# GPUs/goVideoCompressor

Measured on AMD Instinct MI355X. Metric: encoded frames/sec (whole node), 1080p30->H.264 CRF23, higher is better.
Workload: dtype uint8 (8-bit 4:2:0 samples, int32 transforms)

## Files before the change

### csrc/common/h264_cabac.h

```cpp
#pragma once
#include <cstddef>
#include <cstdint>

#include "h264_cabac_tables.h"
#include "h264_mb.h"
#include "h264_tables.h"

namespace mivc {
namespace h264 {

#if defined(__HIPCC__) && defined(__HIP_DEVICE_COMPILE__)
MIVC_HD int cabac_clz32(uint32_t v) { return __clz(static_cast<int>(v)); }
#else
MIVC_HD int cabac_clz32(uint32_t v) { return v ? __builtin_clz(v) : 32; }
#endif

struct CabacBuf {
  uint8_t* p;
  size_t cap;
  size_t n;
  int overflow;
  MIVC_HD void put(int b) {
    if (n < cap) p[n] = static_cast<uint8_t>(b);
    else overflow = 1;
// ... 453 lines not shown
    if (!((cbp >> b8) & 1)) continue;
    const int x4 = (b8 & 1) * 2, y4 = (b8 >> 1) * 2;
    if (n.t8x8) {
      n.cbf_luma |= static_cast<uint16_t>(0x33u << (x4 + 4 * y4));
      continue;
    }
    for (int b4 = 0; b4 < 4; ++b4) {
      const int blk = b8 * 4 + b4;
      if ((mask >> blk) & 1u) n.cbf_luma |= static_cast<uint16_t>(1u << (kBlkX[blk] + 4 * kBlkY[blk]));
    }
  }
}

MIVC_HD void cabac_qp_chain(const CabacSliceInfo& si, CabacNb* nb, int n) {
  int last_qp = si.slice_qp, last_nz = 0;
  for (int a = si.first_mb; a < si.first_mb + n; ++a) {
    CabacNb& m = nb[a];
    const bool has = !m.skip && (m.cbp != 0 || m.kind == MBK_I16x16);
    m.prev_dqp_nz = static_cast<uint8_t>(last_nz);
    if (has) {
      int d = m.qp - last_qp;
      if (d < -26) d += 52;
      if (d > 25) d -= 52;
      m.dqp = static_cast<int8_t>(d);
      last_qp = m.qp;
      last_nz = d != 0;
    } else {
      m.dqp = 0;
      last_nz = 0;
    }
  }
}

template <class E>
struct CabacMbCoder {
  E& e;
  const CabacSliceInfo& si;
  const CabacNb* nb;
  CabacView v;
  const CabacNb* cur;

  MIVC_HD CabacMbCoder(E& e_, const CabacSliceInfo& s, const CabacNb* table) : e(e_), si(s), nb(table), cur(nullptr) {}

  MIVC_HD const CabacNb* nb_mb(int x4, int y4) const {
    const int a = v.mb_of(x4, y4);
    return a < 0 ? nullptr : &nb[a];
  }
  MIVC_HD const CabacNb* A() const { return nb_mb(-1, 0); }
  MIVC_HD const CabacNb* B() const { return nb_mb(0, -1); }

  MIVC_HD void put_mb_skip(int skip) {
    const CabacNb* a = A();
    const CabacNb* b = B();
    const int inc = (a && !a->skip) + (b && !b->skip);
    e.decision((si.slice_type == SLICE_B ? CTX_MB_SKIP_B : CTX_MB_SKIP_P) + inc, skip);
  }

  MIVC_HD void put_mb_type_i(int kind, int i16_mode, int cbp, bool islice) {
    if (islice) {
      const CabacNb* a = A();
      const CabacNb* b = B();
      const int inc = (a && a->kind != MBK_I4x4 && a->kind != MBK_I8x8) + (b && b->kind != MBK_I4x4 && b->kind != MBK_I8x8);
      e.decision(CTX_MB_TYPE_I + inc, kind == MBK_I4x4 || kind == MBK_I8x8 ? 0 : 1);
    } else {
      const int off = si.slice_type == SLICE_B ? CTX_MB_TYPE_B_INTRA : CTX_MB_TYPE_P_INTRA;
      e.decision(off, kind == MBK_I4x4 || kind == MBK_I8x8 ? 0 : 1);
    }
    if (kind == MBK_I4x4 || kind == MBK_I8x8) return;
    e.terminate(kind == MBK_IPCM ? 1 : 0);
    if (kind == MBK_IPCM) return;
    const int cl = (cbp & 15) ? 1 : 0, cc = cbp >> 4;
    if (islice) {
      e.decision(CTX_MB_TYPE_I + 3, cl);
      e.decision(CTX_MB_TYPE_I + 4, cc != 0);
      if (cc) e.decision(CTX_MB_TYPE_I + 5, cc == 2);
      e.decision(CTX_MB_TYPE_I + 6, (i16_mode >> 1) & 1);
      e.decision(CTX_MB_TYPE_I + 7, i16_mode & 1);
    } else {
      const int off = si.slice_type == SLICE_B ? CTX_MB_TYPE_B_INTRA : CTX_MB_TYPE_P_INTRA;
      e.decision(off + 1, cl);
      e.decision(off + 2, cc != 0);
      if (cc) e.decision(off + 2, cc == 2);
      e.decision(off + 3, (i16_mode >> 1) & 1);
      e.decision(off + 3, i16_mode & 1);
    }
  }

  MIVC_HD void put_mb_type_p(int kind, int i16_mode, int cbp) {
    switch (kind) {
      case MBK_P16x16: e.decision(14, 0); e.decision(15, 0); e.decision(16, 0); return;
      case MBK_P16x8:  e.decision(14, 0); e.decision(15, 1); e.decision(17, 1); return;
      case MBK_P8x16:  e.decision(14, 0); e.decision(15, 1); e.decision(17, 0); return;
      case MBK_P8x8:   e.decision(14, 0); e.decision(15, 0); e.decision(16, 1); return;
      default:
        e.decision(14, 1);
        put_mb_type_i(kind, i16_mode, cbp, false);
    }
  }

  MIVC_HD void put_mb_type_b(int kind, int i16_mode, int cbp, int code) {
    const CabacNb* a = A();
    const CabacNb* b = B();
    const int inc = (a && !a->skip && a->kind != MBK_BDIRECT) + (b && !b->skip && b->kind != MBK_BDIRECT);
    if (code == 0) {
      e.decision(CTX_MB_TYPE_B + inc, 0);
      return;
    }
    e.decision(CTX_MB_TYPE_B + inc, 1);
    if (code <= 2) {
      e.decision(CTX_MB_TYPE_B + 3, 0);
      e.decision(CTX_MB_TYPE_B + 5, code - 1);
      return;
    }
    e.decision(CTX_MB_TYPE_B + 3, 1);
    if (code <= 10) {
      const int v3 = code - 3;
      e.decision(CTX_MB_TYPE_B + 4, 0);
      e.decision(CTX_MB_TYPE_B + 5, (v3 >> 2) & 1);
      e.decision(CTX_MB_TYPE_B + 5, (v3 >> 1) & 1);
      e.decision(CTX_MB_TYPE_B + 5, v3 & 1);
      return;
    }
    e.decision(CTX_MB_TYPE_B + 4, 1);
    if (code == 11 || code == 22 || code == 23) {
      e.decision(CTX_MB_TYPE_B + 5, 1);
      e.decision(CTX_MB_TYPE_B + 5, code == 23 ? 0 : 1);
      e.decision(CTX_MB_TYPE_B + 5, code == 11 ? 0 : 1);
      if (code == 23) put_mb_type_i(kind, i16_mode, cbp, false);
      return;
    }
    const int v4 = code - 12;
    e.decision(CTX_MB_TYPE_B + 5, (v4 >> 3) & 1);
    e.decision(CTX_MB_TYPE_B + 5, (v4 >> 2) & 1);
    e.decision(CTX_MB_TYPE_B + 5, (v4 >> 1) & 1);
    e.decision(CTX_MB_TYPE_B + 5, v4 & 1);
  }

  MIVC_HD void put_sub_mb_type_b(int code) {
    if (code == 0) { e.decision(CTX_SUB_MB_B, 0); return; }
    e.decision(CTX_SUB_MB_B, 1);
    if (code <= 2) {
      e.decision(CTX_SUB_MB_B + 1, 0);
      e.decision(CTX_SUB_MB_B + 3, code - 1);
      return;
    }
    e.decision(CTX_SUB_MB_B + 1, 1);
    if (code <= 6) {
      e.decision(CTX_SUB_MB_B + 2, 0);
      e.decision(CTX_SUB_MB_B + 3, ((code - 3) >> 1) & 1);
      e.decision(CTX_SUB_MB_B + 3, (code - 3) & 1);
      return;
    }
    e.decision(CTX_SUB_MB_B + 2, 1);
    if (code >= 11) {
      e.decision(CTX_SUB_MB_B + 3, 1);
      e.decision(CTX_SUB_MB_B + 3, code - 11);
      return;
    }
    e.decision(CTX_SUB_MB_B + 3, 0);
    e.decision(CTX_SUB_MB_B + 3, ((code - 7) >> 1) & 1);
    e.decision(CTX_SUB_MB_B + 3, (code - 7) & 1);
  }

  MIVC_HD void put_ref_idx(int list, int q, int ref) {
    const int x4 = (q & 1) * 2, y4 = (q >> 1) * 2;
    auto cond = [&](int xn, int yn) -> int {
      const CabacNb* m = nb_mb(xn, yn);
      if (!m || m->skip || mbk_is_intra(m->kind)) return 0;
      const int qn = CabacView::quad_of(xn, yn);
      if ((m->direct >> qn) & 1) return 0;
      return m->ref[list][qn] > 0;
    };
    const int inc = cond(x4 - 1, y4) + 2 * cond(x4, y4 - 1);
    e.decision(CTX_REF_IDX + inc, ref > 0);
    if (ref == 0) return;
    for (int k = 1; k < ref; ++k) e.decision(CTX_REF_IDX + (k == 1 ? 4 : 5), 1);
    e.decision(CTX_REF_IDX + (ref == 1 ? 4 : 5), 0);
  }

  MIVC_HD void put_mvd(int list, int q, int comp, int val) {
    const int x4 = (q & 1) * 2, y4 = (q >> 1) * 2;
    auto absn = [&](int xn, int yn) -> int {
      const CabacNb* m = nb_mb(xn, yn);
      if (!m) return 0;
      const int d = m->mvd[list][CabacView::quad_of(xn, yn)][comp];
      return d < 0 ? -d : d;
    };
    const int sum = absn(x4 - 1, y4) + absn(x4, y4 - 1);
    const int base = comp ? CTX_MVD_Y : CTX_MVD_X;
    const int inc0 = sum < 3 ? 0 : (sum > 32 ? 2 : 1);
    const int av = val < 0 ? -val : val;
    const int pre = av < 9 ? av : 9;
    e.decision(base + inc0, pre > 0);
    if (pre > 0) {
      for (int k = 1; k < pre; ++k) e.decision(base + (k < 4 ? k + 2 : 6), 1);
      if (pre < 9) e.decision(base + (pre < 4 ? pre + 2 : 6), 0);
      if (av >= 9) e.bypass_eg(static_cast<uint32_t>(av - 9), 3);
      e.bypass(val < 0);
    }
  }

  MIVC_HD void put_cbp(int cbp) {
    const CabacNb* a = A();
    const CabacNb* b = B();
    const int la = a ? (a->kind == MBK_IPCM ? 0x2F : a->cbp) : 0x0F;
    const int lb = b ? (b->kind == MBK_IPCM ? 0x2F : b->cbp) : 0x0F;
    for (int b8 = 0; b8 < 4; ++b8) {
      const int ca = (b8 & 1) ? ((cbp >> (b8 - 1)) & 1) : ((la >> (b8 + 1)) & 1);
      const int cb = (b8 & 2) ? ((cbp >> (b8 - 2)) & 1) : ((lb >> (b8 + 2)) & 1);
      e.decision(CTX_CBP_LUMA + (ca ? 0 : 1) + 2 * (cb ? 0 : 1), (cbp >> b8) & 1);
    }
    const int ca = a ? (a->kind == MBK_IPCM ? 2 : (a->cbp >> 4)) : 0;
    const int cb = b ? (b->kind == MBK_IPCM ? 2 : (b->cbp >> 4)) : 0;
    const int cc = cbp >> 4;
    e.decision(CTX_CBP_CHROMA + (ca > 0) + 2 * (cb > 0), cc > 0);
    if (cc) e.decision(CTX_CBP_CHROMA + 4 + (ca == 2) + 2 * (cb == 2), cc == 2);
  }

  MIVC_HD void put_qp_delta(int d, int prev_nz) {
    const int m = d > 0 ? 2 * d - 1 : -2 * d;
    e.decision(CTX_QP_DELTA + (prev_nz ? 1 : 0), m > 0);
    if (m > 0) {
      for (int k = 1; k < m; ++k) e.decision(CTX_QP_DELTA + (k == 1 ? 2 : 3), 1);
      e.decision(CTX_QP_DELTA + (m == 1 ? 2 : 3), 0);
    }
  }

  MIVC_HD void put_chroma_mode(int mode) {
    const CabacNb* a = A();
    const CabacNb* b = B();
    const int inc = (a && mbk_is_intra(a->kind) && a->kind != MBK_IPCM && a->chroma_mode != 0) +
                    (b && mbk_is_intra(b->kind) && b->kind != MBK_IPCM && b->chroma_mode != 0);
    e.decision(CTX_CHROMA_PRED + inc, mode > 0);
    if (mode > 0) {
      e.decision(CTX_CHROMA_PRED + 3, mode > 1);
      if (mode > 1) e.decision(CTX_CHROMA_PRED + 3, mode > 2);
    }
  }

  MIVC_HD int pred_intra_mode(int x4, int y4) const {
    const CabacNb* a = nb_mb(x4 - 1, y4);
    const CabacNb* b = nb_mb(x4, y4 - 1);
    if (!a || !b) return 2;
    const int ma = (a->kind == MBK_I4x4 || a->kind == MBK_I8x8) ? a->i4[CabacView::rast_of(x4 - 1, y4)] : 2;
    const int mb = (b->kind == MBK_I4x4 || b->kind == MBK_I8x8) ? b->i4[CabacView::rast_of(x4, y4 - 1)] : 2;
    return ma < mb ? ma : mb;
  }
  MIVC_HD void put_intra_mode(int mode, int pred) {
    if (mode == pred) {
      e.decision(CTX_PREV_INTRA, 1);
      return;
    }
    e.decision(CTX_PREV_INTRA, 0);
    const int rem = mode < pred ? mode : mode - 1;
    e.decision(CTX_REM_INTRA, rem & 1);
    e.decision(CTX_REM_INTRA, (rem >> 1) & 1);
    e.decision(CTX_REM_INTRA, (rem >> 2) & 1);
  }

  MIVC_HD void put_t8x8(int flag) {
    const CabacNb* a = A();
    const CabacNb* b = B();
    e.decision(CTX_T8x8 + (a && a->t8x8) + (b && b->t8x8), flag);
  }

  MIVC_HD void put_block(const int16_t* c, int n, int cat, int cbf_inc, bool nonzero) {
    if (!nonzero) {
      if (cbf_inc >= 0) e.decision(CTX_CBF + kCbfCatOffset[cat] + cbf_inc, 0);
      return;
    }
    int last = -1;
    for (int i = 0; i < n; ++i)
      if (c[i]) last = i;
    if (cbf_inc >= 0) {
      e.decision(CTX_CBF + kCbfCatOffset[cat] + cbf_inc, last >= 0);
      if (last < 0) return;
    }
    for (int i = 0; i < n - 1; ++i) {
      const int sig = c[i] != 0;
      int sctx, lctx;
      if (cat == 5) {
        sctx = CTX_SIG8x8 + kSig8x8Frame[i];
        lctx = CTX_LAST8x8 + kLast8x8Frame[i];
      } else {
        const int inc = cat == 3 ? (i < 2 ? i : 2) : i;
        sctx = CTX_SIG + kSigCatOffset[cat] + inc;
        lctx = CTX_LAST + kSigCatOffset[cat] + inc;
      }
      e.decision(sctx, sig);
      if (sig) {
        e.decision(lctx, i == last);
        if (i == last) break;
      }
    }
    const int abase = cat == 5 ? CTX_ABS8x8 : CTX_ABS + kAbsCatOffset[cat];
    const int gmax = cat == 3 ? 3 : 4;
    int ngt1 = 0, neq1 = 0;
    for (int i = last; i >= 0; --i) {
      const int val = c[i];
      if (!val) continue;
      const int a1 = (val < 0 ? -val : val) - 1;
      e.decision(abase + (ngt1 ? 0 : (neq1 + 1 < 4 ? neq1 + 1 : 4)), a1 > 0);
      if (a1 > 0) {
        const int ctx1 = abase + 5 + (ngt1 < gmax ? ngt1 : gmax);
        const int pre = a1 < 14 ? a1 : 14;
        for (int k = 1; k < pre; ++k) e.decision(ctx1, 1);
        if (pre < 14) e.decision(ctx1, 0);
        else e.bypass_eg(static_cast<uint32_t>(a1 - 14), 0);
        ++ngt1;
      } else {
        ++neq1;
      }
      e.bypass(val < 0);
    }
  }

  MIVC_HD int cbf_luma_inc(int x4, int y4, bool intra) const {
    auto cond = [&](int xn, int yn) -> int {
      const CabacNb* m = nb_mb(xn, yn);
      if (!m) return intra ? 1 : 0;
      if (m->kind == MBK_IPCM) return 1;
      return (m->cbf_luma >> CabacView::rast_of(xn, yn)) & 1;
    };
    return cond(x4 - 1, y4) + 2 * cond(x4, y4 - 1);
  }
  MIVC_HD int cbf_dc_inc(int bit, bool intra) const {
    auto cond = [&](const CabacNb* m) -> int {
      if (!m) return intra ? 1 : 0;
      if (m->kind == MBK_IPCM) return 1;
      return (m->cbf_dc >> bit) & 1;
    };
    return cond(A()) + 2 * cond(B());
  }
  MIVC_HD int cbf_cac_inc(int comp, int cx, int cy, bool intra) const {
    auto cond = [&](const CabacNb* m, int blk) -> int {
      if (!m) return intra ? 1 : 0;
      if (m->kind == MBK_IPCM) return 1;
      return (m->cbf_cac[comp] >> blk) & 1;
    };
    const int a = cx > 0 ? cond(cur, cy * 2) : cond(A(), cy * 2 + 1);
    const int b = cy > 0 ? cond(cur, cx) : cond(B(), 2 + cx);
    return a + 2 * b;
  }

  MIVC_HD void put_inter_pred(const MbHeader& h, int kind) {
    if (kind == MBK_BDIRECT) return;
    const bool bslice = si.slice_type == SLICE_B;
    const CabacParts P = cabac_parts(kind);
    const bool sub8 = P.np == 4;
    const int dir_mask = cur->direct;
    if (sub8) {
      if (bslice) {
        for (int s = 0; s < 4; ++s) {
          int code = 0;
          if (!((dir_mask >> s) & 1)) {
            const bool l0 = h.ref[0][s] >= 0, l1 = h.ref[1][s] >= 0;
            code = (l0 && l1) ? 3 : (l1 ? 2 : 1);
          }
          put_sub_mb_type_b(code);
        }
      } else {
        for (int s = 0; s < 4; ++s) e.decision(CTX_SUB_MB_P, 1);
      }
    }
    for (int l = 0; l < 2; ++l) {
      if (si.num_ref[l] <= 1) continue;
      for (int p = 0; p < P.np; ++p) {
        const int q = P.qfirst(p);
        if (((dir_mask >> q) & 1) || h.ref[l][q] < 0) continue;
        put_ref_idx(l, q, h.ref[l][q]);
      }
    }
    for (int l = 0; l < 2; ++l)
      for (int p = 0; p < P.np; ++p) {
        const int q = P.qfirst(p);
        if (((dir_mask >> q) & 1) || h.ref[l][q] < 0) continue;
        put_mvd(l, q, 0, cur->mvd[l][q][0]);
        put_mvd(l, q, 1, cur->mvd[l][q][1]);
      }
  }

  MIVC_HD void code_mb(int addr, const MbHeader& h, const int16_t* c, bool last_in_slice) {
    v.at(addr, si.wmb, si.first_mb);
    cur = &nb[addr];
    const bool pslice = si.slice_type == SLICE_P, bslice = si.slice_type == SLICE_B;
    if (pslice || bslice) put_mb_skip(cur->skip);
    if (!cur->skip) code_mb_layer(h, c);
    e.terminate(last_in_slice ? 1 : 0);
  }

  MIVC_HD void code_mb_layer(const MbHeader& h, const int16_t* c) {
    const bool pslice = si.slice_type == SLICE_P, bslice = si.slice_type == SLICE_B;
    const int kind = cur->kind;
    const int cbp = cur->cbp;
    const uint32_t mask = cur->mask;
    const bool intra = mbk_is_intra(kind);
    if (pslice) put_mb_type_p(kind, h.i16_mode, cbp);
    else if (bslice) put_mb_type_b(kind, h.i16_mode, cbp, intra ? 23 : cur->b_code);
    else put_mb_type_i(kind, h.i16_mode, cbp, true);
    if (kind == MBK_I4x4 || kind == MBK_I8x8) {
      if (si.t8x8_mode) put_t8x8(kind == MBK_I8x8);
      if (kind == MBK_I4x4) {
        for (int blk = 0; blk < 16; ++blk) {
          const int x4 = kBlkX[blk], y4 = kBlkY[blk];
          put_intra_mode(h.i4_modes[blk], pred_intra_mode(x4, y4));
        }
      } else {
        for (int b8 = 0; b8 < 4; ++b8) put_intra_mode(h.i4_modes[b8 * 4], pred_intra_mode((b8 & 1) * 2, (b8 >> 1) * 2));
      }
    }
    if (intra) put_chroma_mode(h.chroma_mode);
    else put_inter_pred(h, kind);
    if (kind != MBK_I16x16) {
      put_cbp(cbp);
      if ((cbp & 15) && si.t8x8_mode && !intra) put_t8x8(cur->t8x8);
    }
    if (cbp == 0 && kind != MBK_I16x16) return;
    put_qp_delta(cur->dqp, cur->prev_dqp_nz);
    if (kind == MBK_I16x16) put_block(c + COEF_LUMA_DC, 16, 0, cbf_dc_inc(0, true), (mask & NZ_LUMA_DC) != 0);
    for (int b8 = 0; b8 < 4; ++b8) {
      if (!((cbp >> b8) & 1)) continue;
      if (cur->t8x8) {
        put_block(c + COEF_LUMA + b8 * 64, 64, 5, -1, true);
        continue;
      }
      for (int b4 = 0; b4 < 4; ++b4) {
        const int blk = b8 * 4 + b4;
        const int inc = cbf_luma_inc(kBlkX[blk], kBlkY[blk], intra);
        const bool nzb = (mask >> blk) & 1u;
        if (kind == MBK_I16x16) put_block(c + COEF_LUMA + blk * 16 + 1, 15, 1, inc, nzb);
        else put_block(c + COEF_LUMA + blk * 16, 16, 2, inc, nzb);
      }
    }
    const int cc = cbp >> 4;
    if (cc)
      for (int comp = 0; comp < 2; ++comp)
        put_block(c + COEF_CHROMA_DC + comp * 4, 4, 3, cbf_dc_inc(1 + comp, intra), ((mask >> (17 + comp)) & 1u) != 0);
    if (cc == 2)
      for (int comp = 0; comp < 2; ++comp)
        for (int b = 0; b < 4; ++b)
          put_block(c + COEF_CHROMA_AC + (comp * 4 + b) * 16 + 1, 15, 4, cbf_cac_inc(comp, b & 1, b >> 1, intra),
                    ((mask >> (19 + comp * 4 + b)) & 1u) != 0);
  }
};

MIVC_HD void cabac_code_symbol(CabacEncoder& e, uint16_t s) {
  if (!(s & 0x8000u)) e.decision(s & 0x1FF, (s >> 9) & 1);
  else if (!(s & 0x4000u)) e.bypass_bits(s & 0x3FFu, (s >> 10) & 15);
  else e.terminate(s & 1);
}

template <class Out>
struct CabacSymbolCoder {
  uint64_t low;
  uint32_t range;
  int nbits, bad;
  Out out;

  MIVC_HD void init() {
    low = 0;
    range = 510;
    nbits = -1;
    bad = 0;
  }
  MIVC_HD void drain() {
    while (nbits >= 8) {
      const int sh = nbits + 2;
      const uint32_t v = static_cast<uint32_t>(low >> sh);
      low &= (1ull << sh) - 1ull;
      nbits -= 8;
      if (!out.byte9(v)) bad = 1;
    }
  }
  MIVC_HD void step_nodrain(uint32_t sym, uint8_t* st, int stride, const uint8_t* lps, const uint8_t* trans) {
// ... 156 lines not shown
```

### csrc/kernels/bindings_hip.cc

```cpp
#include <pybind11/pybind11.h>
#include <pybind11/stl.h>

#include <cstdint>
#include <stdexcept>
#include <string>
#include <vector>

#include "../common/hevc_ctu_coder.h"
#include "launch.h"
#include "route.h"

namespace py = pybind11;
using mivc::gpu::kExactMaxRows;
using mivc::gpu::kMaxCols;
using mivc::gpu::kMaxRows;

namespace {
template <class T>
T* P(uintptr_t p) {
  return reinterpret_cast<T*>(p);
}
void* S(uintptr_t s) { return reinterpret_cast<void*>(s); }

void limit(const char* entry, const char* what, int n, int most) {
// ... 673 lines not shown
    a.ctb_ops = P<uint32_t>(Q("ctb_ops"));
    a.refs = P<uint8_t>(Q("refs"));
    a.ref_base = P<int32_t>(Q("ref_base"));
    a.slices = P<uint8_t>(Q("slices"));
    a.slice_base = P<int32_t>(Q("slice_base"));
    a.scaling = P<uint8_t>(Q("scaling"));
    a.max_tus = static_cast<int>(I("max_tus"));
    a.err = P<int>(Q("err"));
    if (p.contains("out")) {
      const std::vector<uintptr_t> out = p["out"].cast<std::vector<uintptr_t>>();
      for (int c = 0; c < 3; ++c) a.out[c] = reinterpret_cast<void*>(out.at(c));
      a.out_u8 = static_cast<int>(I("out_u8"));
      a.Fo = static_cast<int>(I("Fo"));
      a.out_w = static_cast<int>(I("out_w"));
      a.out_h = static_cast<int>(I("out_h"));
      a.crop_x = static_cast<int>(I("crop_x"));
      a.crop_y = static_cast<int>(I("crop_y"));
      a.disp = P<int16_t>(Q("disp"));
    }
    if (!a.cur || !a.run || !a.meta || !a.mvf || !a.err) throw std::runtime_error("hevc_decode_stage: null pointer");
    const int r = mivc_launch_hevc_decode(&a, stage, S(stream));
    if (r != 0) throw std::runtime_error("hevc_decode_stage: launch failed (" + std::to_string(r) + ")");
  });
  m.def("cavlc_mb_bytes", []() { return mivc_cavlc_mb_bytes(); });
  m.def("cabac_nb_bytes", []() { return mivc_cabac_nb_bytes(); });
  m.def("cabac_gap", []() { return mivc_cabac_gap(); });
  m.def("cabac_bin", [](int B, int wmb, int hmb, uintptr_t hdr, uintptr_t coef, uintptr_t mask, uintptr_t nb,
                        uintptr_t cnt, uintptr_t off, uintptr_t tot, uintptr_t pool, long long pool_cap,
                        uintptr_t pool_used, uintptr_t base, uintptr_t total, uintptr_t slot_qp, int slice_type,
                        int num_ref_l0, int num_ref_l1, int t8x8_mode, uintptr_t err, uintptr_t stream, uintptr_t route,
                        int slice_rows, uintptr_t pre) {
    if (pre && !route) throw std::invalid_argument("cabac_bin: pre needs the step's route");
    if ((pool & 15) != 0) throw std::invalid_argument("cabac_bin: symbol pool must be 16-byte aligned");
    if (B < 1 || wmb < 1 || hmb < 1) throw std::invalid_argument("cabac_bin: bad geometry");
    mivc_launch_cabac_bin(B, wmb, hmb, P<void>(hdr), P<int16_t>(coef), P<uint32_t>(mask), P<void>(nb), P<int>(cnt),
                          P<long long>(off), P<int>(tot), P<uint16_t>(pool), pool_cap, P<long long>(pool_used),
                          P<long long>(base), P<int>(total), P<int>(slot_qp), slice_type, num_ref_l0, num_ref_l1,
                          t8x8_mode, P<int>(err), S(stream), P<void>(route), slice_rows, P<uint32_t>(pre));
  }, py::arg("B"), py::arg("wmb"), py::arg("hmb"), py::arg("hdr"), py::arg("coef"), py::arg("mask"), py::arg("nb"),
     py::arg("cnt"), py::arg("off"), py::arg("tot"), py::arg("pool"), py::arg("pool_cap"), py::arg("pool_used"),
     py::arg("base"), py::arg("total"), py::arg("slot_qp"), py::arg("slice_type"), py::arg("num_ref_l0"),
     py::arg("num_ref_l1"), py::arg("t8x8_mode"), py::arg("err"), py::arg("stream"), py::arg("route") = 0,
     py::arg("slice_rows") = 0, py::arg("pre") = 0);
  m.def("cabac_code", [](int L, int B, uintptr_t pool, uintptr_t base, uintptr_t total, uintptr_t hdr_bits,
                         uintptr_t hdr_nbits, uintptr_t slot_qp, unsigned long long itypes, uintptr_t bytes,
                         uintptr_t out, uintptr_t out_off, uintptr_t err, uintptr_t stream, uintptr_t host_out,
                         long long host_cap) {
    if (B < 1 || L < 1 || L % B != 0 || L / B > 64) throw std::invalid_argument("cabac_code: L must be G * B, G <= 64");
    if ((out & 15) || (host_out & 15)) throw std::invalid_argument("cabac_code: output buffers must be 16-byte aligned");
    mivc_launch_cabac_code(L, B, P<uint16_t>(pool), P<long long>(base), P<int>(total), P<uint32_t>(hdr_bits),
                           P<int>(hdr_nbits), P<int>(slot_qp), itypes, P<int>(bytes), P<uint8_t>(out),
                           P<long long>(out_off), P<int>(err), P<uint8_t>(host_out), host_cap, S(stream));
  });
  m.def("cavlc", [](int B, int wmb, int hmb, uintptr_t hdr, uintptr_t coef, uintptr_t mbs, uintptr_t len, uintptr_t off,
                    uintptr_t trail, uintptr_t total_bits, uintptr_t slot_bytes, uintptr_t words, long long cap_words,
                    uintptr_t hdr_bits, uintptr_t hdr_nbits, int pslice, int slice_qp, uintptr_t slot_qp,
                    uintptr_t out, uintptr_t out_off, uintptr_t stream, uintptr_t nz) {
    mivc_launch_cavlc(B, wmb, hmb, P<void>(hdr), P<int16_t>(coef), P<void>(mbs), P<int>(len), P<long long>(off),
                      P<int>(trail), P<long long>(total_bits), P<int>(slot_bytes), P<uint32_t>(words), cap_words,
                      P<uint32_t>(hdr_bits), P<int>(hdr_nbits), pslice, slice_qp, P<int>(slot_qp), P<uint8_t>(out),
                      P<long long>(out_off), P<uint8_t>(nz), S(stream));
  }, py::arg("B"), py::arg("wmb"), py::arg("hmb"), py::arg("hdr"), py::arg("coef"), py::arg("mbs"), py::arg("len"),
     py::arg("off"), py::arg("trail"), py::arg("total_bits"), py::arg("slot_bytes"), py::arg("words"),
     py::arg("cap_words"), py::arg("hdr_bits"), py::arg("hdr_nbits"), py::arg("pslice"), py::arg("slice_qp"),
     py::arg("slot_qp"), py::arg("out"), py::arg("out_off"), py::arg("stream"), py::arg("nz") = 0);
  m.def("sse", [](int B, int W, int H, int w, int h, uintptr_t sy, uintptr_t su, uintptr_t sv, uintptr_t ry,
// ... 41 lines not shown
```

### csrc/kernels/cabac.hip

```cpp
#include "kcommon.h"
#include "launch.h"
#include "../common/h264_cabac.h"

namespace mivc {
namespace gpu {

using h264::CabacNb;
using h264::CabacSliceInfo;
using h264::MbHeader;

constexpr int kCabacGap = 64;
constexpr int kArithReadAhead = 160;

struct CabacBinArgs {
  Geom g;
  const MbHeader* hdr;
  const int16_t* coef;
  uint32_t* mask;
  CabacNb* nb;
  int* cnt;
  long long* off;
  int* tot;
  uint16_t* pool;
  long long pool_cap;
// ... 163 lines not shown
  for (int i = i0; i < i1; ++i) loc += a.cnt[base + i];
  const long long incl = wave_scan_add(loc);
  long long p = incl - loc;
  for (int i = i0; i < i1; ++i) {
    a.off[base + i] = p;
    p += a.cnt[base + i];
  }
  if (lane == 63) a.tot[blockIdx.x] = static_cast<int>(incl);
}

__global__ __launch_bounds__(64) void cabac_alloc(CabacBinArgs a) {
  const int B = a.g.B * a.per_slot, lane = threadIdx.x;
  const int per = (B + 63) / 64;
  const int i0 = lane * per, i1 = min(B, i0 + per);
  auto region = [&](int s) { return (static_cast<long long>(a.tot[s]) + kCabacGap + 7) & ~7ll; };
  long long loc = 0;
  for (int i = i0; i < i1; ++i) loc += region(i);
  const long long incl = wave_scan_add(loc);
  const long long sum = __shfl(incl, 63, 64);
  long long p = incl - loc;
  const long long start = *a.pool_used;
  const bool fits = start + sum + kArithReadAhead <= a.pool_cap;
  for (int i = i0; i < i1; ++i) {
    a.base[i] = start + p;
    a.total[i] = fits ? a.tot[i] : -1;
    p += region(i);
  }
  if (lane == 0) {
    if (fits) *a.pool_used = start + sum;
    else atomicOr(a.err, 4);
  }
}

struct StagedEmit {
  uint16_t* g;
  uint16_t* lds;
  long long start;
  long long pos;
  int n;
  __device__ __forceinline__ void emit(uint16_t s) {
    lds[pos & 7] = s;
    ++pos;
    ++n;
    if ((pos & 7) == 0) {
      const long long c0 = pos - 8;
      if (c0 >= start) {
        const uint32_t* w = reinterpret_cast<const uint32_t*>(lds);
        *reinterpret_cast<uint4*>(g + c0) = make_uint4(w[0], w[1], w[2], w[3]);
      } else {
        for (long long i = start; i < pos; ++i) g[i] = lds[i & 7];
      }
    }
  }
  __device__ __forceinline__ void finish() {
    const long long c0 = pos & ~7ll;
    for (long long i = c0 > start ? c0 : start; i < pos; ++i) g[i] = lds[i & 7];
  }
};

__global__ __launch_bounds__(64) __attribute__((amdgpu_waves_per_eu(6, 8))) void cabac_bins(CabacBinArgs a) {
  __shared__ __attribute__((aligned(16))) uint16_t stage[64 * 8];
  const int mb = blockIdx.x * 64 + threadIdx.x, slot = blockIdx.y, n = a.g.nmb();
  if (mb >= n) return;
  const int ls = slice_index(a, slot, mb);
  if (a.total[ls] < 0) return;
  const CabacSliceInfo si = slice_info(a, slot, mb);
  const size_t base = static_cast<size_t>(slot) * n;
  h264::CabacSymbolPacker<StagedEmit> s;
  s.out.g = a.pool + a.base[ls] + kCabacGap;
  s.out.lds = stage + threadIdx.x * 8;
  s.out.start = s.out.pos = a.off[base + mb];
  s.out.n = 0;
  h264::CabacMbCoder<h264::CabacSymbolPacker<StagedEmit>> coder(s, si, a.nb + base);
  coder.code_mb(mb, a.hdr[base + mb], a.coef + (base + mb) * h264::kCoefPerMb, mb == slice_end(a, mb) - 1);
  s.flush_bypass();
  s.out.finish();
}

struct CabacCodeArgs {
  int L;
  int B;
  int lpw;
  uint16_t* pool;
  const long long* base;
  const int* total;
  const uint32_t* hdr_bits;
  const int* hdr_nbits;
  const int* slot_qp;
  unsigned long long itypes;
  int* bytes;
  uint8_t* out;
  long long* out_off;
  int* err;
  uint8_t* host_out;
  long long host_cap;
};

struct RingOut {
  uint8_t* p;
  uint8_t* ring;
  long long n, flushed, cap;
  long long arith0;
  long long hold;
  int ovf;
  __device__ void start(long long header_bytes) {
    arith0 = header_bytes;
    hold = -1;
  }
  __device__ void flush_words() {
// ... 271 lines not shown
```

Before: 17690.

## Vectorize CABAC neighbor and coefficient loads, drop LDS staging for symbol emits

Neighbor macroblock context is loaded once per MB as 16-byte heads into registers instead of repeated byte loads through pointers. Coefficient blocks are loaded as wide vectors and turned into a nonzero bitmap that drives the significance and level loops, with packed nibble tables for 8x8 contexts. The LDS-staged 16-byte symbol writer is replaced by plain per-symbol global stores. This trades scattered scalar loads and LDS traffic for more registers and uncoalesced 2-byte stores, and adds alignment requirements on coef and nb.

Result: no change. 17830 (median of 2 runs) (+0.8%).

```diff
diff --git a/csrc/common/h264_cabac.h b/csrc/common/h264_cabac.h
--- a/csrc/common/h264_cabac.h
+++ b/csrc/common/h264_cabac.h
@@ -509,6 +509,109 @@
   }
 }
 
+MIVC_HD uint32_t cabac_load32(const void* p) {
+#if defined(__HIPCC__) && defined(__HIP_DEVICE_COMPILE__)
+  return *static_cast<const uint32_t*>(p);
+#else
+  uint32_t v;
+  __builtin_memcpy(&v, p, 4);
+  return v;
+#endif
+}
+
+struct CabacLevelWindow {
+  uint32_t w0, w1, w2, w3, w4, w5, w6, w7;
+  MIVC_HD void load16(const int16_t* row) {
+#if defined(__HIPCC__) && defined(__HIP_DEVICE_COMPILE__)
+    const uint4 a = reinterpret_cast<const uint4*>(row)[0];
+    const uint4 b = reinterpret_cast<const uint4*>(row)[1];
+    w0 = a.x; w1 = a.y; w2 = a.z; w3 = a.w;
+    w4 = b.x; w5 = b.y; w6 = b.z; w7 = b.w;
+#else
+    uint32_t t[8];
+    __builtin_memcpy(t, row, 32);
+    w0 = t[0]; w1 = t[1]; w2 = t[2]; w3 = t[3];
+    w4 = t[4]; w5 = t[5]; w6 = t[6]; w7 = t[7];
+#endif
+  }
+  MIVC_HD void load4(const int16_t* quad) {
+#if defined(__HIPCC__) && defined(__HIP_DEVICE_COMPILE__)
+    const uint2 a = *reinterpret_cast<const uint2*>(quad);
+    w0 = a.x; w1 = a.y;
+#else
+    uint32_t t[2];
+    __builtin_memcpy(t, quad, 8);
+    w0 = t[0]; w1 = t[1];
+#endif
+    w2 = w3 = w4 = w5 = w6 = w7 = 0;
+  }
+  static MIVC_HD uint32_t nz2(uint32_t w) { return ((w & 0xFFFFu) ? 1u : 0u) | ((w >> 16) ? 2u : 0u); }
+  MIVC_HD uint32_t nzmap() const {
+    return nz2(w0) | (nz2(w1) << 2) | (nz2(w2) << 4) | (nz2(w3) << 6) | (nz2(w4) << 8) | (nz2(w5) << 10) |
+           (nz2(w6) << 12) | (nz2(w7) << 14);
+  }
+  MIVC_HD int level(int i) const {
+    const uint32_t a0 = (i & 2) ? w1 : w0, a1 = (i & 2) ? w3 : w2, a2 = (i & 2) ? w5 : w4, a3 = (i & 2) ? w7 : w6;
+    const uint32_t b0 = (i & 4) ? a1 : a0, b1 = (i & 4) ? a3 : a2;
+    const uint32_t c = (i & 8) ? b1 : b0;
+    return static_cast<int16_t>((i & 1) ? (c >> 16) : (c & 0xFFFFu));
+  }
+};
+
+constexpr uint64_t cabac_pack_nibbles(const uint8_t* t, int first, int n) {
+  uint64_t v = 0;
+  for (int i = 0; i < 16 && first + i < n; ++i) v |= static_cast<uint64_t>(t[first + i] & 15u) << (4 * i);
+  return v;
+}
+MIVC_HD int cabac_nibble_row(int i, uint64_t r0, uint64_t r1, uint64_t r2, uint64_t r3) {
+  const uint64_t a = (i & 16) ? r1 : r0, b = (i & 16) ? r3 : r2;
+  return static_cast<int>((((i & 32) ? b : a) >> (4 * (i & 15))) & 15u);
+}
+MIVC_HD int cabac_sig8x8_inc(int i) {
+  constexpr uint64_t r0 = cabac_pack_nibbles(kSig8x8Frame, 0, 63), r1 = cabac_pack_nibbles(kSig8x8Frame, 16, 63),
+                     r2 = cabac_pack_nibbles(kSig8x8Frame, 32, 63), r3 = cabac_pack_nibbles(kSig8x8Frame, 48, 63);
+  return cabac_nibble_row(i, r0, r1, r2, r3);
+}
+MIVC_HD int cabac_last8x8_inc(int i) {
+  constexpr uint64_t r0 = cabac_pack_nibbles(kLast8x8Frame, 0, 63), r1 = cabac_pack_nibbles(kLast8x8Frame, 16, 63),
+                     r2 = cabac_pack_nibbles(kLast8x8Frame, 32, 63), r3 = cabac_pack_nibbles(kLast8x8Frame, 48, 63);
+  return cabac_nibble_row(i, r0, r1, r2, r3);
+}
+
+struct CabacNbHead {
+  uint32_t w0, w1, w2, w3;
+  bool ok;
+  MIVC_HD void load(const CabacNb* m, bool present) {
+#if defined(__HIPCC__) && defined(__HIP_DEVICE_COMPILE__)
+    const uint4 a = *reinterpret_cast<const uint4*>(m);
+    w0 = a.x; w1 = a.y; w2 = a.z; w3 = a.w;
+#else
+    uint32_t t[4];
+    __builtin_memcpy(t, m, 16);
+    w0 = t[0]; w1 = t[1]; w2 = t[2]; w3 = t[3];
+#endif
+    ok = present;
+  }
+  MIVC_HD int kind() const { return (w0 >> 8) & 0xFF; }
+  MIVC_HD int skip() const { return (w0 >> 16) & 0xFF; }
+  MIVC_HD int cbp() const { return w0 >> 24; }
+  MIVC_HD int t8x8() const { return w1 & 0xFF; }
+  MIVC_HD int chroma_mode() const { return (w1 >> 8) & 0xFF; }
+  MIVC_HD int direct() const { return (w1 >> 16) & 0xFF; }
+  MIVC_HD int cbf_dc() const { return w1 >> 24; }
+  MIVC_HD int cbf_luma() const { return w2 & 0xFFFF; }
+  MIVC_HD int cbf_cac(int comp) const { return (w2 >> (16 + 8 * comp)) & 0xFF; }
+};
+static_assert(offsetof(CabacNb, kind) == 1 && offsetof(CabacNb, skip) == 2 && offsetof(CabacNb, cbp) == 3 &&
+                  offsetof(CabacNb, t8x8) == 4 && offsetof(CabacNb, chroma_mode) == 5 &&
+                  offsetof(CabacNb, direct) == 6 && offsetof(CabacNb, cbf_dc) == 7 &&
+                  offsetof(CabacNb, cbf_luma) == 8 && offsetof(CabacNb, cbf_cac) == 10 &&
+                  offsetof(CabacNb, ref) == 12 && offsetof(CabacNb, mvd) % 4 == 0 && offsetof(CabacNb, i16_mode) % 4 == 0 &&
+                  offsetof(CabacNb, b_code) == offsetof(CabacNb, i16_mode) + 1 &&
+                  offsetof(CabacNb, dqp) == offsetof(CabacNb, i16_mode) + 2 &&
+                  offsetof(CabacNb, prev_dqp_nz) == offsetof(CabacNb, i16_mode) + 3 && sizeof(CabacNb) % 16 == 0,
+              "CabacNbHead decodes the leading 16 bytes of CabacNb (little-endian)");
+
 template <class E>
 struct CabacMbCoder {
   E& e;
@@ -516,6 +619,7 @@
   const CabacNb* nb;
   CabacView v;
   const CabacNb* cur;
+  CabacNbHead hc, ha, hb;
 
   MIVC_HD CabacMbCoder(E& e_, const CabacSliceInfo& s, const CabacNb* table) : e(e_), si(s), nb(table), cur(nullptr) {}
 
@@ -523,21 +627,17 @@
     const int a = v.mb_of(x4, y4);
     return a < 0 ? nullptr : &nb[a];
   }
-  MIVC_HD const CabacNb* A() const { return nb_mb(-1, 0); }
-  MIVC_HD const CabacNb* B() const { return nb_mb(0, -1); }
+  MIVC_HD CabacNbHead head_of(int x4, int y4) const { return x4 < 0 ? ha : (y4 < 0 ? hb : hc); }
 
   MIVC_HD void put_mb_skip(int skip) {
-    const CabacNb* a = A();
-    const CabacNb* b = B();
-    const int inc = (a && !a->skip) + (b && !b->skip);
+    const int inc = (ha.ok && !ha.skip()) + (hb.ok && !hb.skip());
     e.decision((si.slice_type == SLICE_B ? CTX_MB_SKIP_B : CTX_MB_SKIP_P) + inc, skip);
   }
 
   MIVC_HD void put_mb_type_i(int kind, int i16_mode, int cbp, bool islice) {
     if (islice) {
-      const CabacNb* a = A();
-      const CabacNb* b = B();
-      const int inc = (a && a->kind != MBK_I4x4 && a->kind != MBK_I8x8) + (b && b->kind != MBK_I4x4 && b->kind != MBK_I8x8);
+      const int inc = (ha.ok && ha.kind() != MBK_I4x4 && ha.kind() != MBK_I8x8) +
+                      (hb.ok && hb.kind() != MBK_I4x4 && hb.kind() != MBK_I8x8);
       e.decision(CTX_MB_TYPE_I + inc, kind == MBK_I4x4 || kind == MBK_I8x8 ? 0 : 1);
     } else {
       const int off = si.slice_type == SLICE_B ? CTX_MB_TYPE_B_INTRA : CTX_MB_TYPE_P_INTRA;
@@ -576,9 +676,7 @@
   }
 
   MIVC_HD void put_mb_type_b(int kind, int i16_mode, int cbp, int code) {
-    const CabacNb* a = A();
-    const CabacNb* b = B();
-    const int inc = (a && !a->skip && a->kind != MBK_BDIRECT) + (b && !b->skip && b->kind != MBK_BDIRECT);
+    const int inc = (ha.ok && !ha.skip() && ha.kind() != MBK_BDIRECT) + (hb.ok && !hb.skip() && hb.kind() != MBK_BDIRECT);
     if (code == 0) {
       e.decision(CTX_MB_TYPE_B + inc, 0);
       return;
@@ -642,11 +740,13 @@
   MIVC_HD void put_ref_idx(int list, int q, int ref) {
     const int x4 = (q & 1) * 2, y4 = (q >> 1) * 2;
     auto cond = [&](int xn, int yn) -> int {
-      const CabacNb* m = nb_mb(xn, yn);
-      if (!m || m->skip || mbk_is_intra(m->kind)) return 0;
+      const CabacNbHead m = head_of(xn, yn);
+      const int a = v.mb_of(xn, yn);
+      const uint32_t row = list == 0 ? m.w3 : cabac_load32(&nb[a < 0 ? v.addr : a].ref[1][0]);
+      if (!m.ok || m.skip() || mbk_is_intra(m.kind())) return 0;
       const int qn = CabacView::quad_of(xn, yn);
-      if ((m->direct >> qn) & 1) return 0;
-      return m->ref[list][qn] > 0;
+      if ((m.direct() >> qn) & 1) return 0;
+      return static_cast<int8_t>((row >> (8 * qn)) & 0xFFu) > 0;
     };
     const int inc = cond(x4 - 1, y4) + 2 * cond(x4, y4 - 1);
     e.decision(CTX_REF_IDX + inc, ref > 0);
@@ -655,15 +755,22 @@
     e.decision(CTX_REF_IDX + (ref == 1 ? 4 : 5), 0);
   }
 
-  MIVC_HD void put_mvd(int list, int q, int comp, int val) {
+  MIVC_HD void put_mvd_pair(int list, int q) {
     const int x4 = (q & 1) * 2, y4 = (q >> 1) * 2;
-    auto absn = [&](int xn, int yn) -> int {
-      const CabacNb* m = nb_mb(xn, yn);
-      if (!m) return 0;
-      const int d = m->mvd[list][CabacView::quad_of(xn, yn)][comp];
-      return d < 0 ? -d : d;
+    auto pair = [&](int xn, int yn) -> uint32_t {
+      const int a = v.mb_of(xn, yn);
+      const uint32_t d = cabac_load32(&nb[a < 0 ? v.addr : a].mvd[list][CabacView::quad_of(xn, yn)][0]);
+      return a < 0 ? 0u : d;
     };
-    const int sum = absn(x4 - 1, y4) + absn(x4, y4 - 1);
+    const uint32_t own = cabac_load32(&cur->mvd[list][q][0]);
+    const uint32_t l = pair(x4 - 1, y4), t = pair(x4, y4 - 1);
+    auto comp_of = [](uint32_t d, int comp) -> int { return static_cast<int16_t>(comp ? (d >> 16) : (d & 0xFFFFu)); };
+    auto mag = [](int d) -> int { return d < 0 ? -d : d; };
+    for (int comp = 0; comp < 2; ++comp)
+      put_mvd(comp, comp_of(own, comp), mag(comp_of(l, comp)) + mag(comp_of(t, comp)));
+  }
+
+  MIVC_HD void put_mvd(int comp, int val, int sum) {
     const int base = comp ? CTX_MVD_Y : CTX_MVD_X;
     const int inc0 = sum < 3 ? 0 : (sum > 32 ? 2 : 1);
     const int av = val < 0 ? -val : val;
@@ -678,17 +785,15 @@
   }
 
   MIVC_HD void put_cbp(int cbp) {
-    const CabacNb* a = A();
-    const CabacNb* b = B();
-    const int la = a ? (a->kind == MBK_IPCM ? 0x2F : a->cbp) : 0x0F;
-    const int lb = b ? (b->kind == MBK_IPCM ? 0x2F : b->cbp) : 0x0F;
+    const int la = ha.ok ? (ha.kind() == MBK_IPCM ? 0x2F : ha.cbp()) : 0x0F;
+    const int lb = hb.ok ? (hb.kind() == MBK_IPCM ? 0x2F : hb.cbp()) : 0x0F;
     for (int b8 = 0; b8 < 4; ++b8) {
       const int ca = (b8 & 1) ? ((cbp >> (b8 - 1)) & 1) : ((la >> (b8 + 1)) & 1);
       const int cb = (b8 & 2) ? ((cbp >> (b8 - 2)) & 1) : ((lb >> (b8 + 2)) & 1);
       e.decision(CTX_CBP_LUMA + (ca ? 0 : 1) + 2 * (cb ? 0 : 1), (cbp >> b8) & 1);
     }
-    const int ca = a ? (a->kind == MBK_IPCM ? 2 : (a->cbp >> 4)) : 0;
-    const int cb = b ? (b->kind == MBK_IPCM ? 2 : (b->cbp >> 4)) : 0;
+    const int ca = ha.ok ? (ha.kind() == MBK_IPCM ? 2 : (ha.cbp() >> 4)) : 0;
+    const int cb = hb.ok ? (hb.kind() == MBK_IPCM ? 2 : (hb.cbp() >> 4)) : 0;
     const int cc = cbp >> 4;
     e.decision(CTX_CBP_CHROMA + (ca > 0) + 2 * (cb > 0), cc > 0);
     if (cc) e.decision(CTX_CBP_CHROMA + 4 + (ca == 2) + 2 * (cb == 2), cc == 2);
@@ -704,10 +809,8 @@
   }
 
   MIVC_HD void put_chroma_mode(int mode) {
-    const CabacNb* a = A();
-    const CabacNb* b = B();
-    const int inc = (a && mbk_is_intra(a->kind) && a->kind != MBK_IPCM && a->chroma_mode != 0) +
-                    (b && mbk_is_intra(b->kind) && b->kind != MBK_IPCM && b->chroma_mode != 0);
+    const int inc = (ha.ok && mbk_is_intra(ha.kind()) && ha.kind() != MBK_IPCM && ha.chroma_mode() != 0) +
+                    (hb.ok && mbk_is_intra(hb.kind()) && hb.kind() != MBK_IPCM && hb.chroma_mode() != 0);
     e.decision(CTX_CHROMA_PRED + inc, mode > 0);
     if (mode > 0) {
       e.decision(CTX_CHROMA_PRED + 3, mode > 1);
@@ -736,46 +839,15 @@
   }
 
   MIVC_HD void put_t8x8(int flag) {
-    const CabacNb* a = A();
-    const CabacNb* b = B();
-    e.decision(CTX_T8x8 + (a && a->t8x8) + (b && b->t8x8), flag);
-  }
-
-  MIVC_HD void put_block(const int16_t* c, int n, int cat, int cbf_inc, bool nonzero) {
-    if (!nonzero) {
-      if (cbf_inc >= 0) e.decision(CTX_CBF + kCbfCatOffset[cat] + cbf_inc, 0);
-      return;
-    }
-    int last = -1;
-    for (int i = 0; i < n; ++i)
-      if (c[i]) last = i;
-    if (cbf_inc >= 0) {
-      e.decision(CTX_CBF + kCbfCatOffset[cat] + cbf_inc, last >= 0);
-      if (last < 0) return;
-    }
-    for (int i = 0; i < n - 1; ++i) {
-      const int sig = c[i] != 0;
-      int sctx, lctx;
-      if (cat == 5) {
-        sctx = CTX_SIG8x8 + kSig8x8Frame[i];
-        lctx = CTX_LAST8x8 + kLast8x8Frame[i];
-      } else {
-        const int inc = cat == 3 ? (i < 2 ? i : 2) : i;
-        sctx = CTX_SIG + kSigCatOffset[cat] + inc;
-        lctx = CTX_LAST + kSigCatOffset[cat] + inc;
-      }
-      e.decision(sctx, sig);
-      if (sig) {
-        e.decision(lctx, i == last);
-        if (i == last) break;
-      }
-    }
-    const int abase = cat == 5 ? CTX_ABS8x8 : CTX_ABS + kAbsCatOffset[cat];
-    const int gmax = cat == 3 ? 3 : 4;
-    int ngt1 = 0, neq1 = 0;
-    for (int i = last; i >= 0; --i) {
-      const int val = c[i];
-      if (!val) continue;
+    e.decision(CTX_T8x8 + (ha.ok && ha.t8x8()) + (hb.ok && hb.t8x8()), flag);
+  }
+
+
+  MIVC_HD void put_levels(const CabacLevelWindow& w, uint32_t map, int first, int abase, int gmax, int& ngt1, int& neq1) {
+    while (map) {
+      const int i = 31 - cabac_clz32(map);
+      map ^= 1u << i;
+      const int val = w.level(i + first);
       const int a1 = (val < 0 ? -val : val) - 1;
       e.decision(abase + (ngt1 ? 0 : (neq1 + 1 < 4 ? neq1 + 1 : 4)), a1 > 0);
       if (a1 > 0) {
@@ -784,39 +856,95 @@
         for (int k = 1; k < pre; ++k) e.decision(ctx1, 1);
         if (pre < 14) e.decision(ctx1, 0);
         else e.bypass_eg(static_cast<uint32_t>(a1 - 14), 0);
-        ++ngt1;
-      } else {
-        ++neq1;
-      }
+      }
+      ngt1 += a1 > 0 ? 1 : 0;
+      neq1 += a1 > 0 ? 0 : 1;
       e.bypass(val < 0);
+    }
+  }
+
+  MIVC_HD void put_block(const int16_t* row, int n, int cat, int cbf_inc, bool nonzero) {
+    if (!nonzero) {
+      e.decision(CTX_CBF + kCbfCatOffset[cat] + cbf_inc, 0);
+      return;
+    }
+    CabacLevelWindow w;
+    if (n == 4) w.load4(row);
+    else w.load16(row);
+    const int first = n == 15 ? 1 : 0;
+    const uint32_t map = (w.nzmap() >> first) & ((1u << n) - 1u);
+    e.decision(CTX_CBF + kCbfCatOffset[cat] + cbf_inc, map != 0);
+    if (!map) return;
+    const int last = 31 - cabac_clz32(map);
+    for (int i = 0; i < n - 1; ++i) {
+      const int sig = (map >> i) & 1u;
+      const int inc = cat == 3 ? (i < 2 ? i : 2) : i;
+      e.decision(CTX_SIG + kSigCatOffset[cat] + inc, sig);
+      if (sig) {
+        e.decision(CTX_LAST + kSigCatOffset[cat] + inc, i == last);
+        if (i == last) break;
+      }
+    }
+    int ngt1 = 0, neq1 = 0;
+    put_levels(w, map, first, CTX_ABS + kAbsCatOffset[cat], cat == 3 ? 3 : 4, ngt1, neq1);
+  }
+
+  MIVC_HD void put_block8x8(const int16_t* row) {
+    uint64_t map = 0;
+    {
+      CabacLevelWindow w0, w1, w2, w3;
+      w0.load16(row);
+      w1.load16(row + 16);
+      w2.load16(row + 32);
+      w3.load16(row + 48);
+      map = static_cast<uint64_t>(w0.nzmap() | (w1.nzmap() << 16)) |
+            (static_cast<uint64_t>(w2.nzmap() | (w3.nzmap() << 16)) << 32);
+    }
+    const uint32_t hi = static_cast<uint32_t>(map >> 32), lo = static_cast<uint32_t>(map);
+    const int last = hi ? 63 - cabac_clz32(hi) : (lo ? 31 - cabac_clz32(lo) : -1);
+    for (int i = 0; i < 63; ++i) {
+      const int sig = static_cast<int>((map >> i) & 1u);
+      e.decision(CTX_SIG8x8 + cabac_sig8x8_inc(i), sig);
+      if (sig) {
+        e.decision(CTX_LAST8x8 + cabac_last8x8_inc(i), i == last);
+        if (i == last) break;
+      }
+    }
+    int ngt1 = 0, neq1 = 0;
+    for (int k = 3; k >= 0; --k) {
+      const uint32_t m = static_cast<uint32_t>(map >> (16 * k)) & 0xFFFFu;
+      if (!m) continue;
+      CabacLevelWindow w;
+      w.load16(row + 16 * k);
+      put_levels(w, m, 0, CTX_ABS8x8, 4, ngt1, neq1);
     }
   }
 
   MIVC_HD int cbf_luma_inc(int x4, int y4, bool intra) const {
     auto cond = [&](int xn, int yn) -> int {
-      const CabacNb* m = nb_mb(xn, yn);
-      if (!m) return intra ? 1 : 0;
-      if (m->kind == MBK_IPCM) return 1;
-      return (m->cbf_luma >> CabacView::rast_of(xn, yn)) & 1;
+      const CabacNbHead m = head_of(xn, yn);
+      if (!m.ok) return intra ? 1 : 0;
+      if (m.kind() == MBK_IPCM) return 1;
+      return (m.cbf_luma() >> CabacView::rast_of(xn, yn)) & 1;
     };
     return cond(x4 - 1, y4) + 2 * cond(x4, y4 - 1);
   }
   MIVC_HD int cbf_dc_inc(int bit, bool intra) const {
-    auto cond = [&](const CabacNb* m) -> int {
-      if (!m) return intra ? 1 : 0;
-      if (m->kind == MBK_IPCM) return 1;
-      return (m->cbf_dc >> bit) & 1;
+    auto cond = [&](const CabacNbHead& m) -> int {
+      if (!m.ok) return intra ? 1 : 0;
+      if (m.kind() == MBK_IPCM) return 1;
+      return (m.cbf_dc() >> bit) & 1;
     };
-    return cond(A()) + 2 * cond(B());
+    return cond(ha) + 2 * cond(hb);
   }
   MIVC_HD int cbf_cac_inc(int comp, int cx, int cy, bool intra) const {
-    auto cond = [&](const CabacNb* m, int blk) -> int {
-      if (!m) return intra ? 1 : 0;
-      if (m->kind == MBK_IPCM) return 1;
-      return (m->cbf_cac[comp] >> blk) & 1;
+    auto cond = [&](const CabacNbHead& m, int blk) -> int {
+      if (!m.ok) return intra ? 1 : 0;
+      if (m.kind() == MBK_IPCM) return 1;
+      return (m.cbf_cac(comp) >> blk) & 1;
     };
-    const int a = cx > 0 ? cond(cur, cy * 2) : cond(A(), cy * 2 + 1);
-    const int b = cy > 0 ? cond(cur, cx) : cond(B(), 2 + cx);
+    const int a = cx > 0 ? cond(hc, cy * 2) : cond(ha, cy * 2 + 1);
+    const int b = cy > 0 ? cond(hc, cx) : cond(hb, 2 + cx);
     return a + 2 * b;
   }
 
@@ -825,7 +953,7 @@
     const bool bslice = si.slice_type == SLICE_B;
     const CabacParts P = cabac_parts(kind);
     const bool sub8 = P.np == 4;
-    const int dir_mask = cur->direct;
+    const int dir_mask = hc.direct();
     if (sub8) {
       if (bslice) {
         for (int s = 0; s < 4; ++s) {
@@ -852,28 +980,35 @@
       for (int p = 0; p < P.np; ++p) {
         const int q = P.qfirst(p);
         if (((dir_mask >> q) & 1) || h.ref[l][q] < 0) continue;
-        put_mvd(l, q, 0, cur->mvd[l][q][0]);
-        put_mvd(l, q, 1, cur->mvd[l][q][1]);
+        put_mvd_pair(l, q);
       }
   }
 
   MIVC_HD void code_mb(int addr, const MbHeader& h, const int16_t* c, bool last_in_slice) {
     v.at(addr, si.wmb, si.first_mb);
     cur = &nb[addr];
+    {
+      const int a = v.mb_of(-1, 0), b = v.mb_of(0, -1);
+      hc.load(cur, true);
+      ha.load(&nb[a < 0 ? addr : a], a >= 0);
+      hb.load(&nb[b < 0 ? addr : b], b >= 0);
+    }
     const bool pslice = si.slice_type == SLICE_P, bslice = si.slice_type == SLICE_B;
-    if (pslice || bslice) put_mb_skip(cur->skip);
-    if (!cur->skip) code_mb_layer(h, c);
+    if (pslice || bslice) put_mb_skip(hc.skip());
+    if (!hc.skip()) code_mb_layer(h, c);
     e.terminate(last_in_slice ? 1 : 0);
   }
 
   MIVC_HD void code_mb_layer(const MbHeader& h, const int16_t* c) {
     const bool pslice = si.slice_type == SLICE_P, bslice = si.slice_type == SLICE_B;
-    const int kind = cur->kind;
-    const int cbp = cur->cbp;
-    const uint32_t mask = cur->mask;
+    const int kind = hc.kind();
+    const int cbp = hc.cbp();
+    const bool t8 = hc.t8x8() != 0;
+    const uint32_t tail = cabac_load32(&cur->i16_mode);
+    const uint32_t mask = cabac_load32(&cur->mask);
     const bool intra = mbk_is_intra(kind);
     if (pslice) put_mb_type_p(kind, h.i16_mode, cbp);
-    else if (bslice) put_mb_type_b(kind, h.i16_mode, cbp, intra ? 23 : cur->b_code);
+    else if (bslice) put_mb_type_b(kind, h.i16_mode, cbp, intra ? 23 : static_cast<int>((tail >> 8) & 0xFFu));
     else put_mb_type_i(kind, h.i16_mode, cbp, true);
     if (kind == MBK_I4x4 || kind == MBK_I8x8) {
       if (si.t8x8_mode) put_t8x8(kind == MBK_I8x8);
@@ -890,22 +1025,22 @@
     else put_inter_pred(h, kind);
     if (kind != MBK_I16x16) {
       put_cbp(cbp);
-      if ((cbp & 15) && si.t8x8_mode && !intra) put_t8x8(cur->t8x8);
+      if ((cbp & 15) && si.t8x8_mode && !intra) put_t8x8(t8);
     }
     if (cbp == 0 && kind != MBK_I16x16) return;
-    put_qp_delta(cur->dqp, cur->prev_dqp_nz);
+    put_qp_delta(static_cast<int8_t>((tail >> 16) & 0xFFu), static_cast<int>(tail >> 24));
     if (kind == MBK_I16x16) put_block(c + COEF_LUMA_DC, 16, 0, cbf_dc_inc(0, true), (mask & NZ_LUMA_DC) != 0);
     for (int b8 = 0; b8 < 4; ++b8) {
       if (!((cbp >> b8) & 1)) continue;
-      if (cur->t8x8) {
-        put_block(c + COEF_LUMA + b8 * 64, 64, 5, -1, true);
+      if (t8) {
+        put_block8x8(c + COEF_LUMA + b8 * 64);
         continue;
       }
       for (int b4 = 0; b4 < 4; ++b4) {
         const int blk = b8 * 4 + b4;
-        const int inc = cbf_luma_inc(kBlkX[blk], kBlkY[blk], intra);
+        const int inc = cbf_luma_inc((b8 & 1) * 2 + (b4 & 1), (b8 >> 1) * 2 + (b4 >> 1), intra);
         const bool nzb = (mask >> blk) & 1u;
-        if (kind == MBK_I16x16) put_block(c + COEF_LUMA + blk * 16 + 1, 15, 1, inc, nzb);
+        if (kind == MBK_I16x16) put_block(c + COEF_LUMA + blk * 16, 15, 1, inc, nzb);
         else put_block(c + COEF_LUMA + blk * 16, 16, 2, inc, nzb);
       }
     }
@@ -916,7 +1051,7 @@
     if (cc == 2)
       for (int comp = 0; comp < 2; ++comp)
         for (int b = 0; b < 4; ++b)
-          put_block(c + COEF_CHROMA_AC + (comp * 4 + b) * 16 + 1, 15, 4, cbf_cac_inc(comp, b & 1, b >> 1, intra),
+          put_block(c + COEF_CHROMA_AC + (comp * 4 + b) * 16, 15, 4, cbf_cac_inc(comp, b & 1, b >> 1, intra),
                     ((mask >> (19 + comp * 4 + b)) & 1u) != 0);
   }
 };
diff --git a/csrc/kernels/bindings_hip.cc b/csrc/kernels/bindings_hip.cc
--- a/csrc/kernels/bindings_hip.cc
+++ b/csrc/kernels/bindings_hip.cc
@@ -729,6 +729,8 @@
                         int slice_rows, uintptr_t pre) {
     if (pre && !route) throw std::invalid_argument("cabac_bin: pre needs the step's route");
     if ((pool & 15) != 0) throw std::invalid_argument("cabac_bin: symbol pool must be 16-byte aligned");
+    if ((coef & 15) != 0) throw std::invalid_argument("cabac_bin: coef must be 16-byte aligned");
+    if ((nb & 15) != 0) throw std::invalid_argument("cabac_bin: nb must be 16-byte aligned");
     if (B < 1 || wmb < 1 || hmb < 1) throw std::invalid_argument("cabac_bin: bad geometry");
     mivc_launch_cabac_bin(B, wmb, hmb, P<void>(hdr), P<int16_t>(coef), P<uint32_t>(mask), P<void>(nb), P<int>(cnt),
                           P<long long>(off), P<int>(tot), P<uint16_t>(pool), pool_cap, P<long long>(pool_used),
diff --git a/csrc/kernels/cabac.hip b/csrc/kernels/cabac.hip
--- a/csrc/kernels/cabac.hip
+++ b/csrc/kernels/cabac.hip
@@ -219,49 +219,23 @@
   }
 }
 
-struct StagedEmit {
-  uint16_t* g;
-  uint16_t* lds;
-  long long start;
-  long long pos;
-  int n;
-  __device__ __forceinline__ void emit(uint16_t s) {
-    lds[pos & 7] = s;
-    ++pos;
-    ++n;
-    if ((pos & 7) == 0) {
-      const long long c0 = pos - 8;
-      if (c0 >= start) {
-        const uint32_t* w = reinterpret_cast<const uint32_t*>(lds);
-        *reinterpret_cast<uint4*>(g + c0) = make_uint4(w[0], w[1], w[2], w[3]);
-      } else {
-        for (long long i = start; i < pos; ++i) g[i] = lds[i & 7];
-      }
-    }
-  }
-  __device__ __forceinline__ void finish() {
-    const long long c0 = pos & ~7ll;
-    for (long long i = c0 > start ? c0 : start; i < pos; ++i) g[i] = lds[i & 7];
-  }
+struct PlainEmit {
+  uint16_t* p;
+  __device__ __forceinline__ void emit(uint16_t s) { *p++ = s; }
 };
 
 __global__ __launch_bounds__(64) __attribute__((amdgpu_waves_per_eu(6, 8))) void cabac_bins(CabacBinArgs a) {
-  __shared__ __attribute__((aligned(16))) uint16_t stage[64 * 8];
   const int mb = blockIdx.x * 64 + threadIdx.x, slot = blockIdx.y, n = a.g.nmb();
   if (mb >= n) return;
   const int ls = slice_index(a, slot, mb);
   if (a.total[ls] < 0) return;
   const CabacSliceInfo si = slice_info(a, slot, mb);
   const size_t base = static_cast<size_t>(slot) * n;
-  h264::CabacSymbolPacker<StagedEmit> s;
-  s.out.g = a.pool + a.base[ls] + kCabacGap;
-  s.out.lds = stage + threadIdx.x * 8;
-  s.out.start = s.out.pos = a.off[base + mb];
-  s.out.n = 0;
-  h264::CabacMbCoder<h264::CabacSymbolPacker<StagedEmit>> coder(s, si, a.nb + base);
+  h264::CabacSymbolPacker<PlainEmit> s;
+  s.out.p = a.pool + a.base[ls] + kCabacGap + a.off[base + mb];
+  h264::CabacMbCoder<h264::CabacSymbolPacker<PlainEmit>> coder(s, si, a.nb + base);
   coder.code_mb(mb, a.hdr[base + mb], a.coef + (base + mb) * h264::kCoefPerMb, mb == slice_end(a, mb) - 1);
   s.flush_bypass();
-  s.out.finish();
 }
 
 struct CabacCodeArgs {
```
